# vliu15/3d-brain-tumor-segmentation

Measured on AMD Instinct MI355X. Metric: training volumes/sec (2ch x 128^3), higher is better.
Workload: dtype f32; 1 GPU; BASELINE configs[1]: 2ch x 128^3, batch 1 per GPU, fp32, full fwd+bwd with Dice+KL+L2 VAE loss + Dice metric + TF-form Adam; CLI-default model (base_filters=32, depth=4, groups=8, reduction=8; 42,174,773 params); parallelism=dp1, global_batch=1

## Files before the change

3d-brain-tumor-segmentation_amd/csrc/conv_igemm.hip:

```cpp
#include <stdlib.h>
#include "common.h"
#include "conv_plan.h"

#define MAXSLOT 8

int bts_prof_on();
void bts_prof_begin(int sym, double flops, hipStream_t stream);
void bts_prof_end(hipStream_t stream);

struct IgemmParams {
  const float* x;
  const float* wp;
  const float* bias;
  float* y;
  int N, Di, Hi, Wi, Cin, ldx;
  int Do, Ho, Wo;
  int Cout, ldy, Npad, KG;
  int ODa, OHa, OWa;
  int os, ooz, ooy, oox;
  int s, loz, loy, lox;
  int IZ, IY, IX;
  int lgTX, lgTY, TZ;
  int ntz, nty, ntx;
  int ntaps, flags;
// ... 1666 lines not shown
  if (bias) c.flags |= IG_FLAG_BIAS;
  c.ws_bytes = workspace_bytes;
  ConvPtrs q = {};
  q.x = x; q.wp = wp_fwd; q.bias = bias; q.y = y; q.ws = workspace;
  return conv_run(c, q, stream);
}
extern "C" long bts_conv3d_fwd_workspace(int kind, int N, int D, int H, int W, int Cin, int Cout) {
  return conv_ws_query(0, kind, N, D, H, W, Cin, Cout);
}

extern "C" int bts_conv3d_bwd_data(int kind, const float* dy, const float* wp_bwd, float* dx, void* workspace,
                                   long workspace_bytes, int N, int D, int H, int W, int Cin, int lddx, int Cout, int lddy,
                                   int flags, hipStream_t stream) {
  ConvCall c;
  const int r = conv_call_of(1, kind, N, D, H, W, Cin, lddx, Cout, lddy, flags, c);
  if (r != BTS_OK) return r;
  c.ws_bytes = workspace_bytes;
  ConvPtrs q = {};
  q.x = dy; q.wp = wp_bwd; q.y = dx; q.ws = workspace;
  return conv_run(c, q, stream);
}
extern "C" long bts_conv3d_bwd_data_workspace(int kind, int N, int D, int H, int W, int Cin, int Cout) {
  return conv_ws_query(1, kind, N, D, H, W, Cin, Cout);
}

extern "C" int bts_conv3d_fwd_can_fuse(int N, int D, int H, int W, int Cin, int Cout) {
  ConvCall c;
  ConvChoice ch;
  if (conv_call_of(0, BTS_CONV_K3S1, N, D, H, W, Cin, Cin, Cout, Cout, 0, c) != BTS_OK) return 0;
  conv_query_view(c);
  c.second = CONV_Y2; c.ld2 = Cout;
  return igemm_accept(c, ch) == BTS_OK;
}
extern "C" int bts_conv3d_fwd_fused2(const float* x, const float* wp_fwd, const float* bias, float* y, const float* wp2,
                                     const float* bias2, float* y2, int N, int D, int H, int W, int Cin, int ldx, int Cout,
                                     int ldy, int ldy2, hipStream_t stream) {
  ConvCall c;
  if (conv_call_of(0, BTS_CONV_K3S1, N, D, H, W, Cin, ldx, Cout, ldy, 0, c) != BTS_OK || ldy2 < Cout || !wp2 || !y2) return BTS_ERR_SHAPE;
  if (bias) c.flags |= IG_FLAG_BIAS;
  c.second = CONV_Y2; c.ld2 = ldy2;
  ConvPtrs q = {};
  q.x = x; q.wp = wp_fwd; q.bias = bias; q.y = y; q.wp2 = wp2; q.bias2 = bias2; q.y2 = y2;
  return conv_run(c, q, stream);
}

extern "C" long bts_gn_workspace(int N, long V, int C, int G, int mode);
extern "C" int bts_gn_stats(const float* x, float* mean, float* rstd, void* workspace, long workspace_bytes, int N, long V, int C,
                            int G, int mode, float eps, hipStream_t stream);
static long gnfuse_partial_bytes(int N, int Do, int Ho, int Wo, int Cout) {
  const long tiles = (long)N * ((Do + 0) ) * ((Ho + 3) / 4) * ((Wo + 7) / 8);
  return tiles * ((npad32(Cout) + 31) / 32) * 2 * (long)sizeof(double) + 64;
}
extern "C" long bts_conv3d_fwd_gn_workspace(int kind, int N, int D, int H, int W, int Cin, int Cout, int G) {
  const long cw = bts_conv3d_fwd_workspace(kind, N, D, H, W, Cin, Cout);
  if (cw < 0) return -1;
  int Do = D, Ho = H, Wo = W;
  if (kind == BTS_CONV_K3S2) { Do = D / 2; Ho = H / 2; Wo = W / 2; }
  if (kind == BTS_CONV_K3S2T) { Do = 2 * D; Ho = 2 * H; Wo = 2 * W; }
  const long gw = bts_gn_workspace(N, (long)Do * Ho * Wo, Cout, G, BTS_GN_SLAB);
  if (gw < 0) return -1;
  const long fused = ((cw + 63) & ~63L) + gnfuse_partial_bytes(N, Do, Ho, Wo, Cout);
  return fused > gw ? fused : gw;
}
static int conv_fwd_gn_impl(int kind, const float* x, const float* wp, const float* bias, float* y, const float* wp2,
                            const float* bias2, float* y2, int ldy2, void* ws, long ws_bytes, int N, int D, int H, int W, int Cin,
                            int ldx, int Cout, int G, float eps, float* mean, float* rstd, hipStream_t stream) {
// ... 112 lines not shown
```

3d-brain-tumor-segmentation_amd/csrc/conv_wino3.hip:

```cpp
#include <stdio.h>
#include <stdlib.h>
#include <type_traits>
#include "common.h"
#include "conv_plan.h"
#include "wino_util.h"

int bts_prof_on();
void bts_prof_begin(int sym, double flops, hipStream_t stream);
void bts_prof_end(hipStream_t stream);

struct W3Params {
  const float* x;
  const float* up;
  const float* bias;
  float* y;
  int N, D, H, W, ldx, Cout, ldy, KG;
  int ntz, nty, ntx;
  int accum;
  double* gnp;
  int gn_G, gn_zt;
  int ksplit, kg_per, Npad;
  float* part;
  int nb, ntiles, tiles_per_xcd;
  int T;
  const float* x2;
  const float* wp2;
  int ld2, KG2;
};

#define W3S 12
#define W3SX 18
#define W3LX 20
#define W3NCOL (W3SX * 6 * 2)
#define W3PL (6 * W3LX * W3S)
#define W3BUF (8 * W3PL)
#define W3NSLOT 6
#define W3EX (4 * 4 * 4 * 64 * 4)
#define W3OFF(j, k) ((((j) * W3LX) + ((k) & 1) * 10 + ((k) >> 1)) * W3S)

template <bool X2>
__global__ __launch_bounds__(256, 1) void w3_kernel(const W3Params p) {
  extern __shared__ __attribute__((aligned(16))) float lds[];
  const int tid = threadIdx.x;
  const int lane = tid & 63;
  const int wave = __builtin_amdgcn_readfirstlane(tid >> 6);
  const int h = lane >> 5, l32 = lane & 31;
  const int ptx = l32 & 7, pty = (l32 >> 3) & 1, ptz = l32 >> 4;
  const int nb_ = p.nb;
  const int xcd_ = blockIdx.x & 7;
  const int seq0 = (blockIdx.x >> 3) * p.T;
  int tiles_left = p.ntiles - xcd_ * p.tiles_per_xcd;
  if (tiles_left > p.tiles_per_xcd) tiles_left = p.tiles_per_xcd;
  const int items_here = tiles_left * nb_;
  if (seq0 >= items_here) return;

  struct Item { int n, tz, ty, tx, cb; };
  auto decode = [&](int seq) {
    Item it;
    it.cb = seq % nb_;
    int b = xcd_ * p.tiles_per_xcd + seq / nb_;
    it.tx = b % p.ntx; b /= p.ntx;
    it.ty = b % p.nty; b /= p.nty;
    it.tz = b % p.ntz;
    it.n = b / p.ntz;
    return it;
  };
  auto advance = [&](Item& it) {
    if (++it.cb < nb_) return;
    it.cb = 0;
    if (++it.tx < p.ntx) return;
    it.tx = 0;
    if (++it.ty < p.nty) return;
    it.ty = 0;
    if (++it.tz < p.ntz) return;
    it.tz = 0;
// ... 97 lines not shown
      asm volatile("s_nop 1" ::: "memory");
    }
    {
      wload(aw[0], wt, stn, 1);
#pragma unroll
      for (int k = 0; k < 4; ++k) t[k] = sub4(c[1][k], c[3][k]);
      wino_yt(t, v[1]);
      wino_mfma16<FIRST>(v[0], aw[2], acc[0]);
      WINO_SCHED_GROUP();
      __builtin_amdgcn_sched_barrier(0);
      commit(lds + (par ^ 1) * W3BUF);
      if (FIRST && tid < 32) bsh[bslot * 32 + tid] = bias_v;
      __syncthreads();
      fetch(f_soff);
    }
    {
      wload(aw[1], wt, stn, 2);
      rd_row(ln, 1);
      rd_row(ln, 2);
#pragma unroll
      for (int k = 0; k < 4; ++k) t[k] = add4(c[1][k], c[2][k]);
      wino_yt(t, v[0]);
      wino_mfma16<FIRST>(v[1], aw[3], acc[3]);
      WINO_SCHED_GROUP();
      __builtin_amdgcn_sched_barrier(0);
      asm volatile("s_nop 1" ::: "memory");
    }
  };

  const bool raw = p.ksplit > 1;
  const int ld = raw ? p.Npad : p.ldy;
  const int clim = raw ? p.Npad : p.Cout;
  const bool acc_in = p.accum && !raw;
  f32x4 wf[2][2], xf[2][2][2];
  __amdgpu_buffer_rsrc_t x2r, w2r;
  unsigned x2o[2], w2o = 0x80000000u;
  auto x2_req = [&](int b, int kg0) {
#pragma unroll
    for (int k = 0; k < 2; ++k)
#pragma unroll
      for (int oz = 0; oz < 2; ++oz) xf[b][k][oz] = bufload(x2r, kg0 + k < p.KG2 ? x2o[oz] : 0x80000000u, (unsigned)(kg0 + k) * 32u);
  };
  auto w2_req = [&](int b, int kg0) {
#pragma unroll
    for (int k = 0; k < 2; ++k) wf[b][k] = bufload(w2r, kg0 + k < p.KG2 ? w2o : 0x80000000u, (unsigned)(kg0 + k) * (unsigned)(p.Npad * 32));
  };
  auto finish = [&](const Item& o, int bslot) {
    const float* obase = raw ? p.part + ((long)blockIdx.z * p.N + o.n) * p.D * p.H * p.W * (long)p.Npad
                             : p.y + (long)o.n * p.D * p.H * p.W * (long)p.ldy;
    const __amdgpu_buffer_rsrc_t yr = __builtin_amdgcn_make_buffer_rsrc((void*)obase, 0, 0x7fffffff, 0x00020000);
    if (X2) {
      const int yy = o.ty * 4 + 2 * pty + (wave >> 1), xx = o.tx * 16 + 2 * ptx + (wave & 1), zb = o.tz * 4 + 2 * ptz;
      x2r = __builtin_amdgcn_make_buffer_rsrc((void*)(p.x2 + (long)o.n * p.D * p.H * p.W * (long)p.ld2), 0, 0x7fffffff, 0x00020000);
      w2r = __builtin_amdgcn_make_buffer_rsrc((void*)p.wp2, 0, (unsigned)p.KG2 * (unsigned)(p.Npad * 32), 0x00020000);
#pragma unroll
      for (int oz = 0; oz < 2; ++oz)
        x2o[oz] = (xx < p.W && yy < p.H && (zb + oz) < p.D) ? (unsigned)(((((zb + oz) * p.H + yy) * p.W + xx) * p.ld2 + 4 * h) * 4) : 0x80000000u;
      w2o = (o.cb * 32 + l32 < p.Cout) ? (unsigned)((h * p.Npad + o.cb * 32 + l32) * 16) : 0x80000000u;
      x2_req(0, 0);
      x2_req(1, 2);
    }
    asm volatile("s_nop 15\n\ts_nop 15\n\ts_nop 15\n\ts_nop 15\n\ts_nop 15" ::: "memory");
#pragma unroll
    for (int g = 0; g < 4; ++g) {
      f32x4 tq[4][2];
#pragma unroll
      for (int b = 0; b < 4; ++b) {
        f32x4 q[4];
#pragma unroll
        for (int k = 0; k < 4; ++k)
          q[k] = f32x4{acc_rd(acc[b][k][4 * g]), acc_rd(acc[b][k][4 * g + 1]), acc_rd(acc[b][k][4 * g + 2]), acc_rd(acc[b][k][4 * g + 3])};
        tq[b][0] = add4(add4(q[0], q[1]), q[2]);
        tq[b][1] = sub4(sub4(q[1], q[2]), q[3]);
      }
#pragma unroll
      for (int ox = 0; ox < 2; ++ox) {
        const f32x4 m0 = add4(add4(tq[0][ox], tq[1][ox]), tq[2][ox]);
        const f32x4 m1 = sub4(sub4(tq[1][ox], tq[2][ox]), tq[3][ox]);
        *reinterpret_cast<f32x4*>(ex + (((wave * 4 + g) * 4 + 0 + ox) * 64 + lane) * 4) = m0;
        *reinterpret_cast<f32x4*>(ex + (((wave * 4 + g) * 4 + 2 + ox) * 64 + lane) * 4) = m1;
      }
      __builtin_amdgcn_sched_barrier(0);
    }
    if (X2) {
      w2_req(0, 0);
      w2_req(1, 2);
      __builtin_amdgcn_sched_barrier(0);
    }
    __syncthreads();
    f32x2 gn_s2 = {0.f, 0.f}, gn_q2 = {0.f, 0.f};
    const bool gn_on = p.gnp != nullptr;
    {
      const int oy = wave >> 1, ox = wave & 1;
      const int zb = o.tz * 4 + 2 * ptz, yy = o.ty * 4 + 2 * pty + oy, xx = o.tx * 16 + 2 * ptx + ox;
      unsigned yo[2];
#pragma unroll
      for (int oz = 0; oz < 2; ++oz) {
        const bool ok = xx < p.W && yy < p.H && (zb + oz) < p.D;
        yo[oz] = ok ? (unsigned)(((((zb + oz) * p.H + yy) * p.W + xx) * ld + o.cb * 32 + 4 * h) * 4) : 0x80000000u;
      }
      f32x4 old[4][2];
#pragma unroll
      for (int g = 0; g < 4; ++g)
#pragma unroll
        for (int oz = 0; oz < 2; ++oz) {
          const bool cok = o.cb * 32 + 8 * g + 4 * h < clim;
          old[g][oz] = bufload(yr, (acc_in && cok) ? yo[oz] + 32u * g : 0x80000000u, 0);
        }
      f32x16 a2[2];
      if (X2) {
        const f32x16 zero16 = {0.f, 0.f, 0.f, 0.f, 0.f, 0.f, 0.f, 0.f, 0.f, 0.f, 0.f, 0.f, 0.f, 0.f, 0.f, 0.f};
        for (int kg0 = 0; kg0 < p.KG2; kg0 += 4) {
#pragma unroll
          for (int b = 0; b < 2; ++b) {
            if (b == 0 || kg0 + 2 < p.KG2) {
#pragma unroll
              for (int k = 0; k < 2; ++k)
#pragma unroll
                for (int j = 0; j < 4; ++j)
#pragma unroll
                  for (int oz = 0; oz < 2; ++oz)
                    a2[oz] = __builtin_amdgcn_mfma_f32_32x32x2f32(wf[b][k][j], xf[b][k][oz][j], (kg0 | b | k | j) ? a2[oz] : zero16, 0, 0, 0);
            }
            if (kg0 + 4 < p.KG2) {
              w2_req(b, kg0 + 4 + 2 * b);
              x2_req(b, kg0 + 4 + 2 * b);
            }
          }
        }
      }
#pragma unroll
      for (int g = 0; g < 4; ++g) {
        f32x4 m[4];
#pragma unroll
        for (int a = 0; a < 4; ++a) m[a] = *reinterpret_cast<const f32x4*>(ex + (((a * 4 + g) * 4 + wave) * 64 + lane) * 4);
        const f32x4 bq = *reinterpret_cast<const f32x4*>(bsh + bslot * 32 + 8 * g + 4 * h);
        f32x4 ov[2];
        ov[0] = add4(add4(add4(m[0], m[1]), m[2]), bq);
        ov[1] = add4(sub4(sub4(m[1], m[2]), m[3]), bq);
        const bool cok = o.cb * 32 + 8 * g + 4 * h < clim;
#pragma unroll
        for (int oz = 0; oz < 2; ++oz) {
          const unsigned off = cok ? yo[oz] : 0x80000000u;
          const bool live = off != 0x80000000u;
          f32x4 w = ov[oz];
          if (X2) w = add4(w, f32x4{a2[oz][4 * g], a2[oz][4 * g + 1], a2[oz][4 * g + 2], a2[oz][4 * g + 3]});
          if (gn_on) {
            const f32x4 tt = live ? w : f32x4{0.f, 0.f, 0.f, 0.f};
            gn_s2 = pk_add(pk_add(gn_s2, tt.xy), tt.zw);
            gn_q2 = pk_fma(tt.zw, tt.zw, pk_fma(tt.xy, tt.xy, gn_q2));
          }
          w = add4(w, old[g][oz]);
          __builtin_amdgcn_raw_buffer_store_b128(__builtin_bit_cast(u32x4, w), yr, off + 32u * g, 0, 0);
        }
      }
    }
    {
      double s0 = 0.0, s1 = 0.0;
      const double* dst = nullptr;
      if (gn_on) {
        const double ds = wave_sum_f64((double)gn_s2.x + (double)gn_s2.y), dq = wave_sum_f64((double)gn_q2.x + (double)gn_q2.y);
        if (lane == 0) { gsh[wave * 2] = ds; gsh[wave * 2 + 1] = dq; }
        __syncthreads();
        const int gn_g = o.tz / p.gn_zt;
        const long B = (long)p.gn_zt * p.nty * p.ntx * nb_;
        const long gn_slot = (((long)(o.tz - gn_g * p.gn_zt) * p.nty + o.ty) * p.ntx + o.tx) * nb_ + o.cb;
        dst = p.gnp + (((long)o.n * p.gn_G + gn_g) * B + gn_slot) * 2;
        s0 = gsh[0] + gsh[2] + gsh[4] + gsh[6];
        s1 = gsh[1] + gsh[3] + gsh[5] + gsh[7];
      }
      const __amdgpu_buffer_rsrc_t gr = __builtin_amdgcn_make_buffer_rsrc((void*)dst, 0, gn_on ? 16 : 0, 0x00020000);
      struct D2 { double a, b; } d2{s0, s1};
      __builtin_amdgcn_raw_buffer_store_b128(__builtin_bit_cast(u32x4, d2), gr, (gn_on && tid == 0) ? 0u : 0x80000000u, 0, 0);
    }
  };

  Item cur = decode(seq0), nxt = cur;
  setup_x(cur);
  wr = wdesc(cur);
  wr_n = wr;
  fetch((unsigned)st0 * 32u);
  wload(aw[0], wr, st0, 1);
  wload(aw[1], wr, st0, 2);
  bias_v = bias_of(cur);
  {
    const __amdgpu_buffer_rsrc_t none = __builtin_amdgcn_make_buffer_rsrc((void*)p.y, 0, 0, 0x00020000);
    f32x4 z = {0.f, 0.f, 0.f, 0.f};
#pragma unroll
    for (int i = 0; i < (X2 ? 20 : 8); ++i) z += bufload(none, 0x80000000u + 16u * i, 0);
#pragma unroll
    for (int i = 0; i < 9; ++i) __builtin_amdgcn_raw_buffer_store_b128(__builtin_bit_cast(u32x4, z), none, 0x80000000u + 16u * i, 0, 0);
    const float dummy = bias_of(cur);
    asm volatile("" ::"v"(dummy));
  }
  commit(lds);
  __syncthreads();
  fetch(st0 + 1 < st1 ? (unsigned)(st0 + 1) * 32u : 0x80000000u);
  rd_row(lds, 1);
  rd_row(lds, 2);
#pragma unroll
  for (int k = 0; k < 4; ++k) t[k] = add4(c[1][k], c[2][k]);
  wino_yt(t, v[0]);
  __builtin_amdgcn_sched_barrier(0);
  asm volatile("s_nop 3" ::: "memory");

  int par = 0;
  for (int it = 0; it < p.T; ++it) {
    const bool have_next = (it + 1 < p.T) && (seq0 + it + 1 < items_here);
    const Item out = cur;
    float bias_n = 0.f;
    if (have_next) {
      advance(nxt);
      wr_n = wdesc(nxt);
    }
    bias_n = bias_of(nxt);
    auto run = [&](auto first_tag, int st) {
      if (st + 2 == st1 && have_next) setup_x(nxt);
      const int f = st + 2;
      const unsigned f_soff = f < st1 ? (unsigned)f * 32u : (have_next ? (unsigned)(st0 + f - st1) * 32u : 0x80000000u);
      const bool last = st + 1 == st1;
      stage(first_tag, st, par, f_soff, last ? wr_n : wr, last ? st0 : st + 1, it & 1);
      par ^= 1;
    };
    run(std::true_type{}, st0);
// ... 7 lines not shown
}

static int w3_enabled() {
  const char* e = getenv("BTS_WINO");
  if (e && atoi(e) == 0) return 0;
  e = getenv("BTS_W3");
  return e ? atoi(e) : 1;
}

static bool w3_plan(W3Plan& q, int N, int D, int H, int W, int Cin, int Cout) {
  if (Cin % 8 != 0 || Cout % 4 != 0 || Cout < 16) return false;
  if (W < 12 || H < 4 || D < 4) return false;
  q.ntz = (D + 3) / 4;
  q.nty = (H + 3) / 4;
  q.ntx = (W + 15) / 16;
  q.nb = (Cout + 31) / 32;
  q.wgs = (long)N * q.ntz * q.nty * q.ntx * q.nb;
  if (q.wgs > 0x7fffffffL / 16) return false;
  wino_split(q, N, D, H, W, Cin, 384, 512);
  return true;
}
long w3_ws_need(const ConvCall& c) {
  W3Plan q;
  return w3_enabled() && w3_plan(q, c.N, c.Di, c.Hi, c.Wi, c.Cin, c.Cout) ? q.need : 0;
}
bool w3_accept(const ConvCall& c, ConvChoice& ch) {
  if (!w3_enabled() || !wino_call_ok(c) || !w3_plan(ch.w, c.N, c.Di, c.Hi, c.Wi, c.Cin, c.Cout)) return false;
  ch.sym = 27;
  if (!wino_plan_ok(c, ch)) return false;
  const long nvox = (long)c.N * c.Di * c.Hi * c.Wi;
  if (c.second == CONV_X2 && ch.w.ksplit == 1 && c.ld2 % 4 == 0 && c.p2_16 &&
      nvox >= conv_env_long("BTS_IGEMM_K1S_MIN", 256 * 256) && ((long)c.Di * c.Hi * c.Wi + 64) * (long)c.ld2 * 4 < 0x7fffffffL)
    ch.second = 0;
  return true;
}

int bts_w3_launch_(const ConvCall& c, const ConvChoice& ch, const ConvPtrs& q, hipStream_t stream) {
  const W3Plan& pl = ch.w;
  const int N = c.N, D = c.Di, H = c.Hi, W = c.Wi, Cin = c.Cin, Cout = c.Cout;
  const float* bias = (c.flags & IG_FLAG_BIAS) ? q.bias : nullptr;
  const int accum = (c.flags & IG_FLAG_ACCUM) ? 1 : 0;
  W3Params p;
  p.x = q.x; p.up = q.wp + 75L * ((long)(Cin / 8) * 2 * (pl.nb * 32) * 4); p.bias = bias; p.y = q.y;
  p.N = N; p.D = D; p.H = H; p.W = W; p.ldx = c.ldx; p.Cout = Cout; p.ldy = c.ldy; p.KG = Cin / 8;
  p.ntz = pl.ntz; p.nty = pl.nty; p.ntx = pl.ntx;
  p.accum = accum;
  p.ksplit = pl.ksplit; p.kg_per = pl.kg_per; p.Npad = pl.nb * 32; p.part = reinterpret_cast<float*>(q.ws);
  p.nb = pl.nb; p.ntiles = N * pl.ntz * pl.nty * pl.ntx; p.tiles_per_xcd = (p.ntiles + 7) / 8;
  p.gnp = pl.gn_zt ? q.gnp : nullptr; p.gn_G = pl.gn_zt ? c.G : 0; p.gn_zt = pl.gn_zt ? pl.gn_zt : 1;
  const bool x2 = c.second == CONV_X2 && ch.second == 0;
  p.x2 = x2 ? q.x2 : nullptr; p.wp2 = x2 ? q.wp2 : nullptr; p.ld2 = x2 ? c.ld2 : 0; p.KG2 = x2 ? Cin / 8 : 0;
  static bool attr_done = false;
  const size_t shmem = (2 * W3BUF + W3EX + 64 + 16) * sizeof(float);
  {
    const long items = (long)p.tiles_per_xcd * pl.nb;
    p.T = 1;
    if (pl.ksplit == 1 && p.KG >= 2) {
      long best = -1;
      for (int t = 1; t <= 8; ++t) {
        const long rounds = ((items + t - 1) / t + 31) / 32;
        const long cost = rounds * (8L * t + 1);
        if (best < 0 || cost <= best) { best = cost; p.T = t; }
      }
      const char* e = getenv("BTS_W3_T");
      if (e && atoi(e) > 0) p.T = atoi(e);
    }
  }
  const long wgs_per_xcd = ((long)p.tiles_per_xcd * pl.nb + p.T - 1) / p.T;
  if (!attr_done) {
    hipError_t e = hipFuncSetAttribute(reinterpret_cast<const void*>(w3_kernel<false>), hipFuncAttributeMaxDynamicSharedMemorySize, 160 * 1024);
    if (e != hipSuccess) return (int)e;
    e = hipFuncSetAttribute(reinterpret_cast<const void*>(w3_kernel<true>), hipFuncAttributeMaxDynamicSharedMemorySize, 160 * 1024);
    if (e != hipSuccess) return (int)e;
    attr_done = true;
  }
  const double flops = 2.0 * 27 * Cin * Cout * (double)N * D * H * W;
  const bool prof = bts_prof_on();
  if (prof) bts_prof_begin(27, flops, stream);
  (void)hipGetLastError();
  if (x2) hipLaunchKernelGGL(w3_kernel<true>, dim3((unsigned)(8L * wgs_per_xcd), 1, 1), dim3(256), shmem, stream, p);
  else hipLaunchKernelGGL(w3_kernel<false>, dim3((unsigned)(8L * wgs_per_xcd), 1, pl.ksplit), dim3(256), shmem, stream, p);
  if (prof) bts_prof_end(stream);
  BTS_LAUNCH_CHECK();
  if (pl.ksplit == 1) return BTS_OK;
  return bts_igemm_reduce_(p.part, bias, q.y, (long)N * D * H * W, Cout, p.Npad, c.ldy, pl.ksplit, bias != nullptr, accum, stream);
}
```

3d-brain-tumor-segmentation_amd/layers/resnet.py:

```python
import os

import torch

from .. import ops
from ._base import Layer, Tensor, as_tensor, check_data_format, current_tape, gn_mode_of
from .group_norm import GroupNormalization


class ResnetBlock(Layer):
    def __init__(self, filters, data_format='channels_last', groups=8, reduction=2, l2_scale=1e-5, name=None):
        super(ResnetBlock, self).__init__(name=name)
        self.data_format = check_data_format(data_format)
        self.config = {'filters': filters, 'data_format': data_format, 'reduction': reduction, 'l2_scale': l2_scale,
                       'groups': groups}
        if filters % reduction != 0:
            raise ValueError('Reduction ratio, {}, must be a factor of number of channels, {}.'.format(reduction, filters))
        self.filters = filters
        self.groups = groups
        self.reduction = reduction
        self.l2_scale = l2_scale
        self.norm1 = self.track(GroupNormalization(groups=groups, axis=-1, beta_initializer='zeros',
                                                   gamma_initializer='ones', beta_regularizer=l2_scale,
                                                   gamma_regularizer=l2_scale, name=self.name + '/gn1',
                                                   semantics=gn_mode_of(data_format)))
# ... 21 lines not shown

    @property
    def trainable_variables(self):
        n1, n2 = self.norm1._params, self.norm2._params
        p = self._params
        return p[:7] + n1 + p[7:9] + n2

    def compute_output_shape(self, input_shape):
        return tuple(input_shape[:-1]) + (self.filters,)

    def __call__(self, inputs, training=None, out=None, fold=None):
        inputs = as_tensor(inputs, data_format=self.data_format)
        if not self.built:
            self.build(tuple(inputs.shape), fold)
        return self.call(inputs, training=training, out=out, fold=fold)

    def call(self, inputs, training=None, out=None, fold=None):
        x = as_tensor(inputs, data_format=self.data_format)
        f, g = self.filters, self.groups
        n, d, h, w, cin = x.shape
        dup_start, dup_shift = fold if fold else (0, 0)
        if cin + dup_shift != self.cin_ref:
            raise ValueError('ResnetBlock built for %d input channels, got %d' % (self.cin_ref, cin + dup_shift))
        v = d * h * w
        K1, K3 = ops.K1, ops.K3S1
        pk = lambda key, kind, role, p, ci, co, folded: self.packed(
            key, kind, role, p, ci, co, cin if folded else None, dup_start if folded else 0, dup_shift if folded else 0)
        wp_pt = pk('pt_f', K1, ops.ROLE_FWD, self.ptwise_k, self.cin_ref, f, True)
        wp_c1 = pk('c1_f', K3, ops.ROLE_FWD, self.conv1_k, self.cin_ref, f, True)
        wp_c2 = pk('c2_f', K3, ops.ROLE_FWD, self.conv2_k, f, f, False)
        slab = self.norm1._mode == ops.GN_SLAB
        m1 = r1 = None
        res = None
        if slab:
            fused = ops.conv_fwd_fused2_gn(x.t, wp_c1, self.conv1_b.t, wp_pt, self.ptwise_b.t, f, g, self.norm1.epsilon)
            if fused is not None:
                c1, res, m1, r1 = fused
        else:
            fused = ops.conv_fwd_fused2(x.t, wp_c1, self.conv1_b.t, wp_pt, self.ptwise_b.t, f)
            if fused is not None:
                c1, res = fused
        main = torch.cuda.current_stream()
        gate = ops.side_stream('gate') if res is None else None

        def gate_branch(res_):
            if res_ is None:
                res_ = ops.conv_fwd(K1, x.t, wp_pt, self.ptwise_b.t, f)
            gap_ = ops.colsum(res_, scale=1.0 / v)
            hbuf_, ch_ = ops.se_mlp_fwd(gap_, self.se_w1.t, self.se_w2.t)
            return res_, gap_, hbuf_, ch_

        if gate is not None:
            gate.wait_stream(main)
            with torch.cuda.stream(gate):
                res, gap, hbuf, ch = gate_branch(None)
            x.t.record_stream(gate)
            for t in (res, gap, hbuf, ch):
                t.record_stream(main)
        if fused is None:
            if slab:
                c1, m1, r1 = ops.conv_fwd_gn(K3, x.t, wp_c1, self.conv1_b.t, f, g, self.norm1.epsilon)
            else:
                c1 = ops.conv_fwd(K3, x.t, wp_c1, self.conv1_b.t, f)
        if gate is None:
            res, gap, hbuf, ch = gate_branch(res)
        if m1 is None:
            m1, r1 = ops.gn_stats(c1, g, self.norm1._mode, self.norm1.epsilon)
        a = ops.gn_apply(c1, self.norm1.gamma.t, self.norm1.beta.t, m1, r1, g, self.norm1._mode, True)
        if slab:
            c2, m2, r2 = ops.conv_fwd_gn(K3, a, wp_c2, self.conv2_b.t, f, g, self.norm2.epsilon)
        else:
            c2 = ops.conv_fwd(K3, a, wp_c2, self.conv2_b.t, f)
            m2, r2 = ops.gn_stats(c2, g, self.norm2._mode, self.norm2.epsilon)
        if gate is not None:
            main.wait_stream(gate)
        if out is None:
            out = Tensor(torch.empty((n, d, h, w, f), dtype=torch.float32, device=x.t.device))
        wsp = self.spatial_k.t.reshape(-1)
        sp = ops.block_epilogue_fwd(res, c2, out.t, wsp, ch, self.norm2.gamma.t, self.norm2.beta.t, m2, r2, g, self.norm2._mode)
        out.cf = self.data_format == 'channels_first'
        tape = current_tape()
        if tape is not None:
            def backward():
                self._backward(x, out, res, gap, hbuf, ch, sp, c1, m1, r1, a, c2, m2, r2, dup_start, dup_shift)
            tape.record(backward)
# ... 122 lines not shown
```

3d-brain-tumor-segmentation_amd/ops.py:

```python
import ctypes
import weakref

import numpy as np
import torch

from ._lib import ERRORS, lib

K1, K3S1, K3S2, K3S2T = 0, 1, 2, 3
ROLE_FWD, ROLE_BWD = 0, 1
FLAG_SIGMOID, FLAG_ACCUM = 1, 2
GN_SLAB, GN_CHANNEL = 0, 1

_workspaces = {}

_CFG = {0: '2,1,4,1', 1: '2,2,4,1', 2: '1,2,2,2', 3: '1,1,2,2', 4: '1,1,4,1'}


_VARIANTS = {33: {1: '<0,5>', 2: '<0,4>', 3: '<1,5>', 4: '<1,4>'},
             32: {1: '<3x3x3>', 2: '<1x1x1>'}}


def kernel_symbol(sym, detail=False):
    var, sym = sym >> 16, sym & 0xffff
    if var and detail and sym in _VARIANTS:
# ... 234 lines not shown
                    raise RuntimeError('bts_conv_pack_desc failed: %s' % ERRORS.get(r, r))
                first += r
            dev = entries[0][3].device
            self.dev = torch.frombuffer(bytearray(host), dtype=torch.uint8).to(dev)
            self.host = host
            self.key, self.n, self.blocks = key, len(entries), first
        lib().call('bts_conv_pack_batch', _p(self.dev), ctypes.cast(self.host, ctypes.c_void_p), self.n, self.blocks, _stream())


def conv_packed_empty(kind, role, cin_slab, cout, device):
    return torch.empty(lib().query('bts_conv_packed_floats', kind, role, cin_slab, cout), dtype=torch.float32, device=device)


def conv_out_shape(kind, x_shape, cout):
    n, d, h, w, _ = x_shape
    if kind == K3S2:
        return (n, d // 2, h // 2, w // 2, cout)
    if kind == K3S2T:
        return (n, 2 * d, 2 * h, 2 * w, cout)
    return (n, d, h, w, cout)


def conv_fwd(kind, x, wp, bias, cout, out=None, sigmoid=False):
    n, d, h, w, cin = x.shape
    if out is None:
        out = torch.empty(conv_out_shape(kind, x.shape, cout), dtype=torch.float32, device=x.device)
    nb = lib().query('bts_conv3d_fwd_workspace', kind, n, d, h, w, cin, cout)
    ws = workspace(nb, x.device) if nb > 0 else None
    lib().call('bts_conv3d_fwd', kind, _p(x), _p(wp), _p(bias), _p(out), _p(ws), nb, n, d, h, w, cin, ld_of(x), cout,
               ld_of(out), FLAG_SIGMOID if sigmoid else 0, _stream())
    return out


def conv_fwd_fused2(x, wp3, bias3, wp1, bias1, cout):
    n, d, h, w, cin = x.shape
    if not lib()._bts_conv3d_fwd_can_fuse(n, d, h, w, cin, cout):
        return None
    c1 = torch.empty((n, d, h, w, cout), dtype=torch.float32, device=x.device)
    res = torch.empty_like(c1)
    lib().call('bts_conv3d_fwd_fused2', _p(x), _p(wp3), _p(bias3), _p(c1), _p(wp1), _p(bias1), _p(res), n, d, h, w, cin,
               ld_of(x), cout, cout, cout, _stream())
    return c1, res


def conv_fwd_gn(kind, x, wp, bias, cout, groups, eps):
    n, d, h, w, cin = x.shape
    y = torch.empty(conv_out_shape(kind, x.shape, cout), dtype=torch.float32, device=x.device)
    mean = torch.empty(n * groups, dtype=torch.float32, device=x.device)
    rstd = torch.empty(n * groups, dtype=torch.float32, device=x.device)
    nb = lib().query('bts_conv3d_fwd_gn_workspace', kind, n, d, h, w, cin, cout, groups)
    ws = workspace(nb, x.device)
    lib().call('bts_conv3d_fwd_gn', kind, _p(x), _p(wp), _p(bias), _p(y), _p(ws), nb, n, d, h, w, cin, ld_of(x), cout, groups,
               float(eps), _p(mean), _p(rstd), _stream())
    return y, mean, rstd


def conv_fwd_fused2_gn(x, wp3, bias3, wp1, bias1, cout, groups, eps):
    n, d, h, w, cin = x.shape
    if not lib()._bts_conv3d_fwd_can_fuse(n, d, h, w, cin, cout):
        return None
    c1 = torch.empty((n, d, h, w, cout), dtype=torch.float32, device=x.device)
    res = torch.empty_like(c1)
    mean = torch.empty(n * groups, dtype=torch.float32, device=x.device)
    rstd = torch.empty(n * groups, dtype=torch.float32, device=x.device)
    nb = lib().query('bts_conv3d_fwd_gn_workspace', K3S1, n, d, h, w, cin, cout, groups)
    ws = workspace(nb, x.device)
    lib().call('bts_conv3d_fwd_fused2_gn', _p(x), _p(wp3), _p(bias3), _p(c1), _p(wp1), _p(bias1), _p(res), _p(ws), nb, n, d, h, w,
               cin, ld_of(x), cout, cout, groups, float(eps), _p(mean), _p(rstd), _stream())
    return c1, res, mean, rstd


def conv_bwd_data(kind, dy, wp_bwd, dx, accumulate):
    n, d, h, w, cin = dx.shape
    cout = dy.shape[4]
    nb = lib().query('bts_conv3d_bwd_data_workspace', kind, n, d, h, w, cin, cout)
    ws = workspace(nb, dy.device) if nb > 0 else None
    lib().call('bts_conv3d_bwd_data', kind, _p(dy), _p(wp_bwd), _p(dx), _p(ws), nb, n, d, h, w, cin, ld_of(dx), cout,
               ld_of(dy), FLAG_ACCUM if accumulate else 0, _stream())
    return dx


def conv_bwd_weight(kind, x, dy, dw, db, dup_start=0, dup_shift=0, accumulate=False):
    n, d, h, w, cin = x.shape
    cout = dy.shape[4]
    nb = lib().query('bts_conv3d_bwd_weight_workspace', kind, n, d, h, w, cin, cout)
    ws = workspace(nb, x.device)
    lib().call('bts_conv3d_bwd_weight', kind, _p(x), _p(dy), _p(dw), _p(db), _p(ws), nb, n, d, h, w, cin, ld_of(x),
               cout, ld_of(dy), dup_start, dup_shift, 1 if accumulate else 0, _stream())


def _conv_bwd_weight_query(name, kind, x, dy):
    n, d, h, w, cin = x.shape
# ... 1073 lines not shown
```

include/bts_hip.h:

```cpp
#ifndef BTS_HIP_H
#define BTS_HIP_H
#include <stdint.h>
#ifdef __cplusplus
extern "C" {
#endif

typedef struct ihipStream_t* bts_stream_t;

#define BTS_OK 0
#define BTS_ERR_SHAPE (-1)
#define BTS_ERR_ALIGN (-2)
#define BTS_ERR_UNSUPPORTED (-3)
#define BTS_ERR_WORKSPACE (-4)
#define BTS_ERR_RCCL_BASE (-100)

#define BTS_CONV_K1 0
#define BTS_CONV_K3S1 1
#define BTS_CONV_K3S2 2
#define BTS_CONV_K3S2T 3
#define BTS_ROLE_FWD 0
#define BTS_ROLE_BWD_DATA 1
#define BTS_CONV_FLAG_SIGMOID 1
#define BTS_CONV_FLAG_ACCUM 2

#define BTS_GN_SLAB 0
#define BTS_GN_CHANNEL 1


long bts_conv_packed_floats(int kind, int role, int Cin, int Cout);
int bts_conv_pack(int kind, int role, const float* w, float* wp, int Cin_ref, int Cout, int Cin_slab, int dup_start,
                  int dup_shift, bts_stream_t stream);
long bts_conv_pack_desc_bytes(void);
long bts_conv_pack_desc(void* host_table, int index, long first_block, int kind, int role, const float* w, float* wp,
                        int Cin_ref, int Cout, int Cin_slab, int dup_start, int dup_shift);
int bts_conv_pack_batch(const void* table_dev, const void* table_host, int n, long total_blocks, bts_stream_t stream);
long bts_conv_pack_generation(void);
int bts_conv_pack_forget(const float* wp);
long bts_conv3d_fwd_workspace(int kind, int N, int D, int H, int W, int Cin, int Cout);
int bts_conv3d_fwd(int kind, const float* x, const float* wp_fwd, const float* bias, float* y, void* workspace,
                   long workspace_bytes, int N, int D, int H, int W, int Cin, int ldx, int Cout, int ldy, int flags,
                   bts_stream_t stream);
int bts_conv3d_fwd_can_fuse(int N, int D, int H, int W, int Cin, int Cout);
int bts_conv3d_fwd_fused2(const float* x, const float* wp_fwd, const float* bias, float* y, const float* wp2,
                          const float* bias2, float* y2, int N, int D, int H, int W, int Cin, int ldx, int Cout, int ldy,
                          int ldy2, bts_stream_t stream);
long bts_conv3d_bwd_data_workspace(int kind, int N, int D, int H, int W, int Cin, int Cout);
int bts_conv3d_bwd_data(int kind, const float* dy, const float* wp_bwd, float* dx, void* workspace, long workspace_bytes,
                        int N, int D, int H, int W, int Cin, int lddx, int Cout, int lddy, int flags, bts_stream_t stream);
int bts_conv3d_fwd_config(int kind, int N, int D, int H, int W, int Cin, int Cout);
int bts_conv3d_bwd_data_config(int kind, int N, int D, int H, int W, int Cin, int Cout);
int bts_conv3d_kernel(int dir, int kind, int N, int D, int H, int W, int Cin, int ldx, int Cout, int ldy, int flags, int second,
                      int ld2, int G, int aligned, long workspace_bytes);
int bts_conv3d_bwd_data_pair_launches(int N, int D, int H, int W, int Cin, int lddx, int Cout, int lddy, int lddy2, int flags,
                                      int aligned, long workspace_bytes);
long bts_conv3d_bwd_weight_workspace(int kind, int N, int D, int H, int W, int Cin, int Cout);
int bts_conv3d_bwd_weight(int kind, const float* x, const float* dy, float* dw, float* db, void* workspace,
                          long workspace_bytes, int N, int D, int H, int W, int Cin, int ldx, int Cout, int lddy,
                          int dup_start, int dup_shift, int accumulate, bts_stream_t stream);
int bts_conv3d_bwd_weight_kernel(int kind, int N, int D, int H, int W, int Cin, int ldx, int Cout, int lddy, int aligned);
int bts_conv3d_bwd_weight_form(int kind, int N, int D, int H, int W, int Cin, int ldx, int Cout, int lddy, int aligned);

long bts_gn_workspace(int N, long V, int C, int G, int mode);
long bts_gn_bwd_workspace(int N, long V, int C, int G, int mode);
int bts_gn_stats(const float* x, float* mean, float* rstd, void* workspace, long workspace_bytes, int N, long V, int C,
                 int G, int mode, float eps, bts_stream_t stream);
int bts_gn_apply(const float* x, float* y, const float* gamma, const float* beta, const float* mean, const float* rstd,
                 int N, long V, int C, int ldy, int G, int mode, int relu, bts_stream_t stream);
int bts_gn_bwd(const float* x, const float* dy, float* dx, const float* gamma, const float* beta, const float* mean,
               const float* rstd, float* dgamma, float* dbeta, void* workspace, long workspace_bytes, int N, long V, int C,
               int lddy, int G, int mode, int relu, int accumulate_params, bts_stream_t stream);

long bts_colsum_workspace(int N, long rows, int C);
int bts_colsum(const float* x, float* out, void* workspace, long workspace_bytes, int N, long rows, int C, int ld,
               float scale, int sum_over_n, int accumulate, bts_stream_t stream);
int bts_se_mlp_fwd(const float* gap, const float* w1, const float* w2, float* h, float* ch, int N, int F, int R,
                   bts_stream_t stream);
int bts_block_epilogue_fwd(const float* res, const float* c2, float* out, float* sp, const float* wsp, const float* ch,
                           const float* gamma, const float* beta, const float* mean, const float* rstd, int N, long V,
// ... 295 lines not shown
```

Baseline: 28.98 volumes/s.

## Fuse pointwise residual conv into Winograd 3x3 forward kernel and overlap gate branch

```diff
diff --git a/3d-brain-tumor-segmentation_amd/csrc/conv_igemm.hip b/3d-brain-tumor-segmentation_amd/csrc/conv_igemm.hip
--- a/3d-brain-tumor-segmentation_amd/csrc/conv_igemm.hip
+++ b/3d-brain-tumor-segmentation_amd/csrc/conv_igemm.hip
@@ -1722,6 +1722,18 @@
   c.second = CONV_Y2; c.ld2 = Cout;
   return igemm_accept(c, ch) == BTS_OK;
 }
+extern "C" int bts_conv3d_fwd_pair_launches(int N, int D, int H, int W, int Cin, int ldx, int Cout, int ldy, int ldy2, int flags, int G,
+                                            int aligned, long workspace_bytes) {
+  ConvCall c;
+  ConvChoice ch;
+  if (conv_call_of(0, BTS_CONV_K3S1, N, D, H, W, Cin, ldx, Cout, ldy, flags, c) != BTS_OK || ldy2 < Cout || G < 0) return BTS_ERR_SHAPE;
+  c.second = CONV_Y2; c.ld2 = ldy2; c.G = G;
+  c.x16 = aligned & 1; c.y16 = (aligned >> 1) & 1; c.p2_16 = (aligned >> 2) & 1; c.ws16 = (aligned >> 3) & 1;
+  c.ws_bytes = workspace_bytes < 0 ? LONG_MAX : workspace_bytes;
+  const int r = conv_choose(c, ch);
+  if (r == BTS_ERR_UNSUPPORTED) return 2;
+  return r != BTS_OK ? r : ch.second ? 2 : 1;
+}
 extern "C" int bts_conv3d_fwd_fused2(const float* x, const float* wp_fwd, const float* bias, float* y, const float* wp2,
                                      const float* bias2, float* y2, int N, int D, int H, int W, int Cin, int ldx, int Cout,
                                      int ldy, int ldy2, hipStream_t stream) {
diff --git a/3d-brain-tumor-segmentation_amd/csrc/conv_wino3.hip b/3d-brain-tumor-segmentation_amd/csrc/conv_wino3.hip
--- a/3d-brain-tumor-segmentation_amd/csrc/conv_wino3.hip
+++ b/3d-brain-tumor-segmentation_amd/csrc/conv_wino3.hip
@@ -26,6 +26,9 @@
   const float* x2;
   const float* wp2;
   int ld2, KG2;
+  float* y2;
+  const float* bias2;
+  int ldy2;
 };
 
 #define W3S 12
@@ -38,9 +41,12 @@
 #define W3EX (4 * 4 * 4 * 64 * 4)
 #define W3OFF(j, k) ((((j) * W3LX) + ((k) & 1) * 10 + ((k) >> 1)) * W3S)
 
-template <bool X2>
+enum { W3_PLAIN = 0, W3_X2 = 1, W3_Y2 = 2 };
+template <int MODE>
 __global__ __launch_bounds__(256, 1) void w3_kernel(const W3Params p) {
   extern __shared__ __attribute__((aligned(16))) float lds[];
+  constexpr bool X2 = MODE != W3_PLAIN;
+  constexpr bool Y2 = MODE == W3_Y2;
   const int tid = threadIdx.x;
   const int lane = tid & 63;
   const int wave = __builtin_amdgcn_readfirstlane(tid >> 6);
@@ -204,7 +210,7 @@
   const int ld = raw ? p.Npad : p.ldy;
   const int clim = raw ? p.Npad : p.Cout;
   const bool acc_in = p.accum && !raw;
-  f32x4 wf[2][2], xf[2][2][2];
+  f32x4 wf[2][2], xf[2][2][2], b2[4];
   __amdgpu_buffer_rsrc_t x2r, w2r;
   unsigned x2o[2], w2o = 0x80000000u;
   auto x2_req = [&](int b, int kg0) {
@@ -257,6 +263,11 @@
     if (X2) {
       w2_req(0, 0);
       w2_req(1, 2);
+      if (Y2) {
+        const __amdgpu_buffer_rsrc_t b2r = __builtin_amdgcn_make_buffer_rsrc((void*)p.bias2, 0, p.bias2 ? (unsigned)p.Cout * 4u : 0u, 0x00020000);
+#pragma unroll
+        for (int g = 0; g < 4; ++g) b2[g] = bufload(b2r, (unsigned)(o.cb * 32 + 8 * g + 4 * h) * 4u, 0);
+      }
       __builtin_amdgcn_sched_barrier(0);
     }
     __syncthreads();
@@ -265,20 +276,25 @@
     {
       const int oy = wave >> 1, ox = wave & 1;
       const int zb = o.tz * 4 + 2 * ptz, yy = o.ty * 4 + 2 * pty + oy, xx = o.tx * 16 + 2 * ptx + ox;
-      unsigned yo[2];
+      unsigned yo[2], y2o[2];
 #pragma unroll
       for (int oz = 0; oz < 2; ++oz) {
         const bool ok = xx < p.W && yy < p.H && (zb + oz) < p.D;
         yo[oz] = ok ? (unsigned)(((((zb + oz) * p.H + yy) * p.W + xx) * ld + o.cb * 32 + 4 * h) * 4) : 0x80000000u;
-      }
+        if (Y2) y2o[oz] = ok ? (unsigned)(((((zb + oz) * p.H + yy) * p.W + xx) * p.ldy2 + o.cb * 32 + 4 * h) * 4) : 0x80000000u;
+      }
+      __amdgpu_buffer_rsrc_t y2r;
+      if (Y2) y2r = __builtin_amdgcn_make_buffer_rsrc((void*)(p.y2 + (long)o.n * p.D * p.H * p.W * (long)p.ldy2), 0, 0x7fffffff, 0x00020000);
       f32x4 old[4][2];
-#pragma unroll
-      for (int g = 0; g < 4; ++g)
-#pragma unroll
-        for (int oz = 0; oz < 2; ++oz) {
-          const bool cok = o.cb * 32 + 8 * g + 4 * h < clim;
-          old[g][oz] = bufload(yr, (acc_in && cok) ? yo[oz] + 32u * g : 0x80000000u, 0);
-        }
+      if (!Y2) {
+#pragma unroll
+        for (int g = 0; g < 4; ++g)
+#pragma unroll
+          for (int oz = 0; oz < 2; ++oz) {
+            const bool cok = o.cb * 32 + 8 * g + 4 * h < clim;
+            old[g][oz] = bufload(yr, (acc_in && cok) ? yo[oz] + 32u * g : 0x80000000u, 0);
+          }
+      }
       f32x16 a2[2];
       if (X2) {
         const f32x16 zero16 = {0.f, 0.f, 0.f, 0.f, 0.f, 0.f, 0.f, 0.f, 0.f, 0.f, 0.f, 0.f, 0.f, 0.f, 0.f, 0.f};
@@ -316,14 +332,18 @@
           const unsigned off = cok ? yo[oz] : 0x80000000u;
           const bool live = off != 0x80000000u;
           f32x4 w = ov[oz];
-          if (X2) w = add4(w, f32x4{a2[oz][4 * g], a2[oz][4 * g + 1], a2[oz][4 * g + 2], a2[oz][4 * g + 3]});
+          if (X2 && !Y2) w = add4(w, f32x4{a2[oz][4 * g], a2[oz][4 * g + 1], a2[oz][4 * g + 2], a2[oz][4 * g + 3]});
           if (gn_on) {
             const f32x4 tt = live ? w : f32x4{0.f, 0.f, 0.f, 0.f};
             gn_s2 = pk_add(pk_add(gn_s2, tt.xy), tt.zw);
             gn_q2 = pk_fma(tt.zw, tt.zw, pk_fma(tt.xy, tt.xy, gn_q2));
           }
-          w = add4(w, old[g][oz]);
+          w = add4(w, Y2 ? f32x4{0.f, 0.f, 0.f, 0.f} : old[g][oz]);
           __builtin_amdgcn_raw_buffer_store_b128(__builtin_bit_cast(u32x4, w), yr, off + 32u * g, 0, 0);
+          if (Y2) {
+            const f32x4 w2 = add4(f32x4{a2[oz][4 * g], a2[oz][4 * g + 1], a2[oz][4 * g + 2], a2[oz][4 * g + 3]}, b2[g]);
+            __builtin_amdgcn_raw_buffer_store_b128(__builtin_bit_cast(u32x4, w2), y2r, (cok ? y2o[oz] : 0x80000000u) + 32u * g, 0, 0);
+          }
         }
       }
     }
@@ -359,9 +379,9 @@
     const __amdgpu_buffer_rsrc_t none = __builtin_amdgcn_make_buffer_rsrc((void*)p.y, 0, 0, 0x00020000);
     f32x4 z = {0.f, 0.f, 0.f, 0.f};
 #pragma unroll
-    for (int i = 0; i < (X2 ? 20 : 8); ++i) z += bufload(none, 0x80000000u + 16u * i, 0);
-#pragma unroll
-    for (int i = 0; i < 9; ++i) __builtin_amdgcn_raw_buffer_store_b128(__builtin_bit_cast(u32x4, z), none, 0x80000000u + 16u * i, 0, 0);
+    for (int i = 0; i < (Y2 ? 16 : X2 ? 20 : 8); ++i) z += bufload(none, 0x80000000u + 16u * i, 0);
+#pragma unroll
+    for (int i = 0; i < (Y2 ? 17 : 9); ++i) __builtin_amdgcn_raw_buffer_store_b128(__builtin_bit_cast(u32x4, z), none, 0x80000000u + 16u * i, 0, 0);
     const float dummy = bias_of(cur);
     asm volatile("" ::"v"(dummy));
   }
@@ -435,6 +455,9 @@
   if (c.second == CONV_X2 && ch.w.ksplit == 1 && c.ld2 % 4 == 0 && c.p2_16 &&
       nvox >= conv_env_long("BTS_IGEMM_K1S_MIN", 256 * 256) && ((long)c.Di * c.Hi * c.Wi + 64) * (long)c.ld2 * 4 < 0x7fffffffL)
     ch.second = 0;
+  if (c.second == CONV_Y2 && ch.w.ksplit == 1 && c.ld2 % 4 == 0 && c.p2_16 && !(c.flags & IG_FLAG_ACCUM) && getenv("BTS_IGEMM_NOPAIR") == nullptr &&
+      nvox >= conv_env_long("BTS_IGEMM_K1S_MIN", 256 * 256) && ((long)c.Di * c.Hi * c.Wi + 64) * (long)c.ld2 * 4 < 0x7fffffffL)
+    ch.second = 0;
   return true;
 }
 
@@ -452,7 +475,9 @@
   p.nb = pl.nb; p.ntiles = N * pl.ntz * pl.nty * pl.ntx; p.tiles_per_xcd = (p.ntiles + 7) / 8;
   p.gnp = pl.gn_zt ? q.gnp : nullptr; p.gn_G = pl.gn_zt ? c.G : 0; p.gn_zt = pl.gn_zt ? pl.gn_zt : 1;
   const bool x2 = c.second == CONV_X2 && ch.second == 0;
-  p.x2 = x2 ? q.x2 : nullptr; p.wp2 = x2 ? q.wp2 : nullptr; p.ld2 = x2 ? c.ld2 : 0; p.KG2 = x2 ? Cin / 8 : 0;
+  const bool y2 = c.second == CONV_Y2 && ch.second == 0;
+  p.x2 = x2 ? q.x2 : y2 ? q.x : nullptr; p.wp2 = x2 || y2 ? q.wp2 : nullptr; p.ld2 = x2 ? c.ld2 : y2 ? c.ldx : 0; p.KG2 = x2 || y2 ? Cin / 8 : 0;
+  p.y2 = y2 ? q.y2 : nullptr; p.bias2 = y2 ? q.bias2 : nullptr; p.ldy2 = y2 ? c.ld2 : 0;
   static bool attr_done = false;
   const size_t shmem = (2 * W3BUF + W3EX + 64 + 16) * sizeof(float);
   {
@@ -471,9 +496,11 @@
   }
   const long wgs_per_xcd = ((long)p.tiles_per_xcd * pl.nb + p.T - 1) / p.T;
   if (!attr_done) {
-    hipError_t e = hipFuncSetAttribute(reinterpret_cast<const void*>(w3_kernel<false>), hipFuncAttributeMaxDynamicSharedMemorySize, 160 * 1024);
+    hipError_t e = hipFuncSetAttribute(reinterpret_cast<const void*>(w3_kernel<W3_PLAIN>), hipFuncAttributeMaxDynamicSharedMemorySize, 160 * 1024);
     if (e != hipSuccess) return (int)e;
-    e = hipFuncSetAttribute(reinterpret_cast<const void*>(w3_kernel<true>), hipFuncAttributeMaxDynamicSharedMemorySize, 160 * 1024);
+    e = hipFuncSetAttribute(reinterpret_cast<const void*>(w3_kernel<W3_X2>), hipFuncAttributeMaxDynamicSharedMemorySize, 160 * 1024);
+    if (e != hipSuccess) return (int)e;
+    e = hipFuncSetAttribute(reinterpret_cast<const void*>(w3_kernel<W3_Y2>), hipFuncAttributeMaxDynamicSharedMemorySize, 160 * 1024);
     if (e != hipSuccess) return (int)e;
     attr_done = true;
   }
@@ -481,8 +508,9 @@
   const bool prof = bts_prof_on();
   if (prof) bts_prof_begin(27, flops, stream);
   (void)hipGetLastError();
-  if (x2) hipLaunchKernelGGL(w3_kernel<true>, dim3((unsigned)(8L * wgs_per_xcd), 1, 1), dim3(256), shmem, stream, p);
-  else hipLaunchKernelGGL(w3_kernel<false>, dim3((unsigned)(8L * wgs_per_xcd), 1, pl.ksplit), dim3(256), shmem, stream, p);
+  if (x2) hipLaunchKernelGGL(w3_kernel<W3_X2>, dim3((unsigned)(8L * wgs_per_xcd), 1, 1), dim3(256), shmem, stream, p);
+  else if (y2) hipLaunchKernelGGL(w3_kernel<W3_Y2>, dim3((unsigned)(8L * wgs_per_xcd), 1, 1), dim3(256), shmem, stream, p);
+  else hipLaunchKernelGGL(w3_kernel<W3_PLAIN>, dim3((unsigned)(8L * wgs_per_xcd), 1, pl.ksplit), dim3(256), shmem, stream, p);
   if (prof) bts_prof_end(stream);
   BTS_LAUNCH_CHECK();
   if (pl.ksplit == 1) return BTS_OK;
diff --git a/3d-brain-tumor-segmentation_amd/layers/resnet.py b/3d-brain-tumor-segmentation_amd/layers/resnet.py
--- a/3d-brain-tumor-segmentation_amd/layers/resnet.py
+++ b/3d-brain-tumor-segmentation_amd/layers/resnet.py
@@ -77,16 +77,19 @@
         slab = self.norm1._mode == ops.GN_SLAB
         m1 = r1 = None
         res = None
+        launches, sym = ops.conv_fwd_pair_launches(x.t, f, g if slab else 0)
+        pair = launches == 1
         if slab:
-            fused = ops.conv_fwd_fused2_gn(x.t, wp_c1, self.conv1_b.t, wp_pt, self.ptwise_b.t, f, g, self.norm1.epsilon)
+            fused = ops.conv_fwd_fused2_gn(x.t, wp_c1, self.conv1_b.t, wp_pt, self.ptwise_b.t, f, g, self.norm1.epsilon, pair=pair)
             if fused is not None:
                 c1, res, m1, r1 = fused
         else:
-            fused = ops.conv_fwd_fused2(x.t, wp_c1, self.conv1_b.t, wp_pt, self.ptwise_b.t, f)
+            fused = ops.conv_fwd_fused2(x.t, wp_c1, self.conv1_b.t, wp_pt, self.ptwise_b.t, f, pair=pair)
             if fused is not None:
                 c1, res = fused
         main = torch.cuda.current_stream()
-        gate = ops.side_stream('gate') if res is None else None
+        behind = res is not None and pair and sym == 27
+        gate = ops.side_stream('gate') if res is None or behind else None
 
         def gate_branch(res_):
             if res_ is None:
@@ -95,7 +98,16 @@
             hbuf_, ch_ = ops.se_mlp_fwd(gap_, self.se_w1.t, self.se_w2.t)
             return res_, gap_, hbuf_, ch_
 
-        if gate is not None:
+        if gate is not None and behind:
+            ev = torch.cuda.Event()
+            ev.record(main)
+            gate.wait_event(ev)
+            with torch.cuda.stream(gate):
+                res, gap, hbuf, ch = gate_branch(res)
+            res.record_stream(gate)
+            for t in (gap, hbuf, ch):
+                t.record_stream(main)
+        elif gate is not None:
             gate.wait_stream(main)
             with torch.cuda.stream(gate):
                 res, gap, hbuf, ch = gate_branch(None)
diff --git a/3d-brain-tumor-segmentation_amd/ops.py b/3d-brain-tumor-segmentation_amd/ops.py
--- a/3d-brain-tumor-segmentation_amd/ops.py
+++ b/3d-brain-tumor-segmentation_amd/ops.py
@@ -290,9 +290,20 @@
     return out
 
 
-def conv_fwd_fused2(x, wp3, bias3, wp1, bias1, cout):
+def conv_fwd_pair_launches(x, cout, groups=0):
     n, d, h, w, cin = x.shape
-    if not lib()._bts_conv3d_fwd_can_fuse(n, d, h, w, cin, cout):
+    nb = 0
+    if groups:
+        nb = (max(lib()._bts_conv3d_fwd_workspace(K3S1, n, d, h, w, cin, cout), 0) + 63) & ~63
+    aligned = (1 if x.data_ptr() % 16 == 0 else 0) | 2 | 4 | 8
+    ld = ld_of(x)
+    return (lib()._bts_conv3d_fwd_pair_launches(n, d, h, w, cin, ld, cout, cout, cout, 0, groups, aligned, nb),
+            lib()._bts_conv3d_kernel(0, K3S1, n, d, h, w, cin, ld, cout, cout, 0, 1, cout, groups, aligned, nb))
+
+
+def conv_fwd_fused2(x, wp3, bias3, wp1, bias1, cout, pair=False):
+    n, d, h, w, cin = x.shape
+    if not pair and not lib()._bts_conv3d_fwd_can_fuse(n, d, h, w, cin, cout):
         return None
     c1 = torch.empty((n, d, h, w, cout), dtype=torch.float32, device=x.device)
     res = torch.empty_like(c1)
@@ -313,9 +324,9 @@
     return y, mean, rstd
 
 
-def conv_fwd_fused2_gn(x, wp3, bias3, wp1, bias1, cout, groups, eps):
+def conv_fwd_fused2_gn(x, wp3, bias3, wp1, bias1, cout, groups, eps, pair=False):
     n, d, h, w, cin = x.shape
-    if not lib()._bts_conv3d_fwd_can_fuse(n, d, h, w, cin, cout):
+    if not pair and not lib()._bts_conv3d_fwd_can_fuse(n, d, h, w, cin, cout):
         return None
     c1 = torch.empty((n, d, h, w, cout), dtype=torch.float32, device=x.device)
     res = torch.empty_like(c1)
diff --git a/include/bts_hip.h b/include/bts_hip.h
--- a/include/bts_hip.h
+++ b/include/bts_hip.h
@@ -44,6 +44,8 @@
 int bts_conv3d_fwd_fused2(const float* x, const float* wp_fwd, const float* bias, float* y, const float* wp2,
                           const float* bias2, float* y2, int N, int D, int H, int W, int Cin, int ldx, int Cout, int ldy,
                           int ldy2, bts_stream_t stream);
+int bts_conv3d_fwd_pair_launches(int N, int D, int H, int W, int Cin, int ldx, int Cout, int ldy, int ldy2, int flags, int G,
+                                 int aligned, long workspace_bytes);
 long bts_conv3d_bwd_data_workspace(int kind, int N, int D, int H, int W, int Cin, int Cout);
 int bts_conv3d_bwd_data(int kind, const float* dy, const float* wp_bwd, float* dx, void* workspace, long workspace_bytes,
                         int N, int D, int H, int W, int Cin, int lddx, int Cout, int lddy, int flags, bts_stream_t stream);
```

Result: no change. 29.09 volumes/s, median of 6 (+0.4%).
